# zhuzilin/ring-flash-attention

Measured on AMD Instinct MI355X. Metric: iters/sec fwd+bwd zigzag_ring, seq=8192*ws, h=32, d=128 bf16, higher is better.
Workload: dtype bf16; 1 GPU; zigzag_ring_flash_attn_kvpacked_func fwd+bwd, per-rank q=(1,8192,32,128) kv=(1,8192,2,8,128) bf16 causal, total seq 8192; kv_heads=8, world_size=1, forward_only=False

## Files before the change

ring-flash-attention_amd/csrc/rfa_bwd.hip:

```cpp
#include <type_traits>

#include "rfa_common.hpp"
#include "rfa_kernels.hpp"

#ifndef RFA_DQ_AHEAD1
#define RFA_DQ_AHEAD1 3
#endif
#ifndef RFA_KV_AHEAD
#define RFA_KV_AHEAD 3
#endif
#ifndef RFA_KV_WIDE_UNROLL
#define RFA_KV_WIDE_UNROLL 1
#endif
#ifndef RFA_KV_AHEAD2
#define RFA_KV_AHEAD2 2
#endif
#ifndef RFA_KV_X_LOAD
#define RFA_KV_X_LOAD 1
#endif
#ifndef RFA_KV_X_LDS
#define RFA_KV_X_LDS 1
#endif
#ifndef RFA_KV_X_VALU
#define RFA_KV_X_VALU 1
#endif
#ifndef RFA_KV_X_SYNC
#define RFA_KV_X_SYNC 1
#endif
#ifndef RFA_KV_PRIO
#define RFA_KV_PRIO 0
#endif
#ifndef RFA_SPILL_AUX
#define RFA_SPILL_AUX 2
#endif
#ifndef RFA_KV_PIN
#define RFA_KV_PIN 1
#endif

namespace rfa {

constexpr int kDqWaves = 8;
constexpr int kDqThreads = kDqWaves * 64;
constexpr int kDqRows = kDqWaves * 32;
constexpr int kDqKV = 64;
template <int kD> constexpr int dq_smem() { return 4 * kDqKV * HeadGeo<kD>::kRowBytes; }

template <typename T, int kD, bool kFullD, bool kWin, bool kDrop = false>
__global__ __launch_bounds__(kDqThreads, 2) void dq_kernel(const BwdParams p) {
  extern __shared__ __attribute__((aligned(16))) char smem_raw[];
  lds_t* smem = (lds_t*)smem_raw;
  typedef HeadGeo<kD> Geo;
  constexpr int kRowBytes = Geo::kRowBytes;
  constexpr int kNK = Geo::kKSteps, kNB = Geo::kDBlocks;
  constexpr int kDqTileBytes = kDqKV * kRowBytes;
  constexpr int kShare = kDqTileBytes / 1024 / kDqWaves;
  constexpr int kChunks = Geo::kLay / 8;
  constexpr int kRowsPerPass = kDqThreads / kChunks;

  const int tid = threadIdx.x;
  const int lane = tid & 63;
  const int wave = __builtin_amdgcn_readfirstlane(tid >> 6);
  const int g = lane >> 5;
  const int l31 = lane & 31;

  int idx = blockIdx.x;
  const int G = p.H / p.Hk;
// ... 387 lines not shown
    const int kr = krow < lk ? krow : lk - 1;
    const T* kp = kbase + (int64_t)kr * p.k_st.row;
#pragma unroll
    for (int kk = 0; kk < kNK; ++kk) {
      const int chunk = 2 * kk + g;
      kwr[kk] = (kFullD || chunk * 8 < p.D) ? *(const vec8<T>*)(kp + chunk * 8) : zero8<T>();
    }
  }

  vec8<T> qreg[kPasses], doreg[kPasses];
  float statreg = 0.f;
  const float stat_scale = (tid & kKvQ) ? -1.f : -kLog2e;
#ifndef RFA_KV_DMA
#define RFA_KV_DMA 1
#endif
  constexpr bool kDma = kFullD && RFA_KV_DMA;
  int voff_q[kPasses], voff_do[kPasses];
#pragma unroll
  for (int i = 0; i < kPasses; ++i) {
    int row = sr + kRowsPerPass * i, chunk = sc;
    if (kDma) dma_lane_src<kD>(wave + kKvWaves * i, lane, row, chunk);
    voff_q[i] = (row * (int)p.q_st.row + chunk * 8) * 2;
    voff_do[i] = (row * (int)p.dout_st.row + chunk * 8) * 2;
  }
  int dma_stage = 0;
  int ld_g = 0, ld_j = jtop > 0 ? jtop : 0;
  int ld_c = 0;
  const int64_t q_tile_e = (int64_t)kKvQ * p.q_st.row, do_tile_e = (int64_t)kKvQ * p.dout_st.row;
  const float* st_base0 = wave ? dltbase0 : lsebase0;
  const int64_t st_head_e = wave ? p.delta_head : p.lse_head;
  const T* ld_q = qbase0 + ld_j * q_tile_e;
  const T* ld_do = dobase0 + ld_j * do_tile_e;
  const float* ld_st = st_base0 + ld_j * kKvQ;
  auto load_tile = [&]() {
    const int j = RFA_KV_X_LOAD == 2 ? 0 : ld_j;
    const T* qtile = RFA_KV_X_LOAD == 2 ? qbase0 : ld_q;
    const T* dotile = RFA_KV_X_LOAD == 2 ? dobase0 : ld_do;
    const float* sttile = ld_st;
    if (++ld_g >= G) {
      ld_g = 0;
      if (kBal) {
        ++ld_c;
        ld_j = ld_c == w_n1 ? w_j2 : (ld_c < w_n1 ? ld_j - 1 : ld_j + 1);
      } else {
        ld_j -= nsplit;
      }
      ld_q = qbase0 + ld_j * q_tile_e;
      ld_do = dobase0 + ld_j * do_tile_e;
      ld_st = st_base0 + ld_j * kKvQ;
    } else {
      ld_q += p.q_st.head;
      ld_do += p.dout_st.head;
      ld_st += st_head_e;
    }
    int rows = lq - j * kKvQ;
    rows = rows < kKvQ ? rows : kKvQ;
    const int nq = rows > 0 ? ((rows - 1) * (int)p.q_st.row + p.D) * 2 : 0;
    const int ndo = rows > 0 ? ((rows - 1) * (int)p.dout_st.row + p.D) * 2 : 0;
    const buf_rsrc_t rq = make_rsrc(qtile, nq);
    const buf_rsrc_t rdo = make_rsrc(dotile, ndo);
    const dma_rsrc_t dq_ = make_dma_rsrc(qtile, nq);
    const dma_rsrc_t ddo = make_dma_rsrc(dotile, ndo);
#pragma unroll
    for (int i = 0; i < kPasses; ++i) {
      if (kDma) {
        const int dst = lds_addr(smem) + dma_stage + (wave + kKvWaves * i) * 1024;
        dma_load128(dq_, dst, voff_q[i]);
        if (RFA_KV_X_LOAD != 3) dma_load128(ddo, dst + kOffDo, voff_do[i]);
      } else {
        qreg[i] = buffer_load128<T>(rq, voff_q[i]);
        doreg[i] = buffer_load128<T>(rdo, voff_do[i]);
        if (!sd_ok) {
          qreg[i] = zero8<T>();
          doreg[i] = zero8<T>();
        }
      }
    }
    if (wave < 2) {
      const dma_rsrc_t rs = make_dma_rsrc(sttile, rows > 0 ? rows * 4 : 0);
      statreg = buffer_load32_async(rs, lane * 4);
    }
    dma_stage ^= kKvTileBytes;
  };
  int wq = lds_addr(smem) + tile_off_d<kD>(sr, sc);
  int ws = lds_addr(smem) + kOffStat + tid * 4;
  auto write_tile = [&]() {
    if (!kDma) {
#pragma unroll
      for (int i = 0; i < kPasses; ++i) {
        lds_write128<T>(lds_ptr(wq) + i * kRowsPerPass * kRowBytes, qreg[i]);
        lds_write128<T>(lds_ptr(wq) + i * kRowsPerPass * kRowBytes + kOffDo, doreg[i]);
      }
    }
    if (tid < 2 * kKvQ) *(__attribute__((address_space(3))) float*)lds_ptr(ws) = statreg * stat_scale;
  };

  int aq = lds_addr(smem) + tile_off_d<kD>(l31, g) + par * 32 * kRowBytes;
  const int av = lds_addr(smem) + tile_off_d<kD>(l31, g) + kOffV + kbw * 32 * kRowBytes;
  int tq[kTK][2];
#pragma unroll
  for (int kv = 0; kv < kTK; ++kv)
#pragma unroll
    for (int hh = 0; hh < 2; ++hh) {
      tq[kv][hh] = lds_addr(smem) + par * 32 * kRowBytes + tr_off_d<kD>(lane, 0, 16 * kv + 8 * hh + 4 * g);
      pin_vgpr(tq[kv][hh]);
    }
  int mask_g4 = 4 * g, mask_kg = krow - 4 * g;
  pin_vgpr(mask_g4); pin_vgpr(mask_kg);
  int sa = lds_addr(smem) + kOffStat + (32 * par + 4 * g) * 4;
  int avp = av;
  pin_vgpr(aq); pin_vgpr(avp); pin_vgpr(sa); pin_vgpr(wq); pin_vgpr(ws);

  const int ds_lane = 16 * (16 * (l31 >> 2) + 4 * g + (l31 & 3));
  const int ds_nkb = ds_blocks(p.Sk, p.k_half);
  const int64_t ds_head_bytes = p.ds_head_blocks * kDsBlockBytes;
  const char* ds_b = kSpill ? (const char*)p.ds + ds_base_blocks(p, b) * kDsBlockBytes + (int64_t)h0 * ds_head_bytes : nullptr;
  const int64_t ds_g0 = (qs.row0 >> 5) + b;
  const int ds_kb = __builtin_amdgcn_readfirstlane(kblk * (kKeys / 32) + kbw);

  const uint32_t drop_j = kDrop ? p.k_pos0 + (uint32_t)(p.cu_k ? ks.row0 : 0) + (uint32_t)krow : 0u;
  const uint32_t drop_i0 = kDrop ? p.q_pos0 + (uint32_t)(p.cu_q ? qs.row0 : 0) : 0u;
  const float c = p.scale * kLog2e;
  f32x16 dk[kNB], dv[kNB];
#pragma unroll
  for (int i = 0; i < kNB; ++i)
#pragma unroll
    for (int r = 0; r < 16; ++r) { dk[i][r] = 0.f; dv[i][r] = 0.f; }

  load_tile();
  wait_all_vmem();
  load_landed(statreg);
  write_tile();
  wq ^= kKvTileBytes;
  ws ^= kKvStatBytes;
  __syncthreads();

#if RFA_KV_PRIO == 1
  if (par == 0) __builtin_amdgcn_s_setprio(2);
#elif RFA_KV_PRIO == 2
  if (wave >= kKvWaves / 2) __builtin_amdgcn_s_setprio(1);
#endif
  const int ntile = ntile_q * G;
  int j = jtop, cg = 0, jc = 0;
  int ds_roff0 = kSpill ? (int)ds_rowpart(p, 2 * j, ds_g0, ds_nkb) : 0;
  int ds_rlen0 = kSpill ? ds_rowlen(p, 2 * j, ds_nkb) : 0;
  const char* ds_hp = ds_b;
  for (int f = 0; f < ntile; ++f) {
    if (RFA_KV_X_LOAD && f + 1 < ntile) load_tile();
    int nact = 0;
    bool active = false;
#if RFA_KV_WIDE_UNROLL
#pragma unroll
#else
#pragma unroll 1
#endif
    for (int t0 = 0; t0 < (kWide ? 2 : 1); ++t0) {
    const int t = kWide ? t0 : par;
    constexpr bool kImm = kWide && RFA_KV_WIDE_UNROLL;
    const int toff = kImm ? t0 * 32 * kRowBytes : 0, soff_t = kImm ? t0 * 32 * 4 : 0;
    const int qs0 = j * kKvQ + 32 * t;
    active = (kw0 < lk) && (qs0 < lq) && !(hi && qs0 + 31 + off + wr < kw0) &&
             !(lo && qs0 + off - wl > kw0 + 31);
    if (active) {
      ++nact;
      f32x16 s, dp;
      if (RFA_KV_PRIO == 3 || RFA_KV_PRIO == 5) __builtin_amdgcn_s_setprio(1);
#pragma unroll
      for (int jj = 0; jj < 4; ++jj) {
        const f32x4 nd = *(__attribute__((address_space(3))) f32x4*)(lds_ptr(sa) + (kKvQ + 8 * jj) * 4 + soff_t);
#pragma unroll
        for (int e = 0; e < 4; ++e) { dp[4 * jj + e] = nd[e]; s[4 * jj + e] = 0.f; }
      }
      {
        constexpr int kAhead = RFA_KV_AHEAD;
        constexpr int kN = 2 * kNK;
        vec8<T> a[kN], w[kNK];
        auto fa = [&](int i) {
          if (!RFA_KV_X_LDS || (RFA_KV_X_LDS == 2 && t0 == 1)) return kwr[i % kNK];
          return lds_read128<T>(lds_ptr(aq ^ ((i % kNK) << 5)) + (i < kNK ? kOffDo : 0) + toff);
        };
        auto fw = [&](int i) {
          if (!RFA_KV_X_LDS || (RFA_KV_X_LDS == 2 && t0 == 1)) return kwr[i];
          return lds_read128<T>(lds_ptr(avp ^ (i << 5)));
        };
#pragma unroll
        for (int i = 0; i < kAhead; ++i) { a[i] = fa(i); w[i] = fw(i); }
#pragma unroll
        for (int i = 0; i < kN; ++i) {
          if (i + kAhead < kN) a[i + kAhead] = fa(i + kAhead);
          if (i + kAhead < kNK) w[i + kAhead] = fw(i + kAhead);
          if (i < kNK) dp = mfma(a[i], w[i], dp);
          else s = mfma(a[i], kwr[i - kNK], s);
// ... 6 lines not shown
          __builtin_amdgcn_sched_group_barrier(0x100, 2, 0);
        }
#pragma unroll
        for (int i = 0; i < kNK; ++i) {
          __builtin_amdgcn_sched_group_barrier(0x008, 1, 0);
          __builtin_amdgcn_sched_group_barrier(0x100, 1, 0);
        }
        __builtin_amdgcn_sched_group_barrier(0x008, kAhead, 0);
#endif
      }
      if (RFA_KV_PRIO == 3 || RFA_KV_PRIO == 5) __builtin_amdgcn_s_setprio(0);
      f32x4 l2v[4];
#pragma unroll
      for (int jj = 0; jj < 4; ++jj) l2v[jj] = *(__attribute__((address_space(3))) f32x4*)(lds_ptr(sa) + 8 * jj * 4 + soff_t);
      const bool need_mask = (qs0 + 32 > lq) || (hi && qs0 + off + wr < kw0 + 31) ||
                             (lo && qs0 + 31 + off - wl > kw0);
#pragma unroll
      for (int jj = 0; jj < 4; ++jj)
#pragma unroll
        for (int e = 0; e < 4; ++e)
          if (RFA_KV_X_VALU) s[4 * jj + e] = fast_exp2(__builtin_fmaf(s[4 * jj + e], c, l2v[jj][e]));
      if (RFA_KV_X_VALU && need_mask) {
#pragma unroll
        for (int r = 0; r < 16; ++r) {
          const int sq = qs0 + crow(r, 0);
          const bool ok = (mask_g4 < lq - sq) & (!hi | (mask_kg <= sq + off + wr)) & (!lo | (mask_kg >= sq + off - wl));
          s[r] = ok ? s[r] : 0.f;
        }
      }
      if (kDrop) {
        const uint32_t hkey = drop_head_key(p.drop_seed, p.cu_q ? 0u : (uint32_t)b, p.head0 + (uint32_t)(h0 + cg));
#pragma unroll
        for (int jj = 0; jj < 4; ++jj) {
          const f32x4 nd = *(__attribute__((address_space(3))) f32x4*)(lds_ptr(sa) + (kKvQ + 8 * jj) * 4);
#pragma unroll
          for (int e = 0; e < 4; ++e) {
            const int r = 4 * jj + e;
            const uint32_t w = drop_word(hkey, drop_i0 + (uint32_t)(qs0 + crow(r, g)), drop_j >> 2);
            const bool keep = drop_keep(w, (int)(drop_j & 3u), p.drop_keep);
            const float dpd = keep ? (dp[r] - nd[e]) * p.drop_scale + nd[e] : nd[e];
            dp[r] = dpd * s[r];
            s[r] = keep ? s[r] * p.drop_scale : 0.f;
          }
        }
      } else {
#pragma unroll
      for (int jj = 0; jj < 4; ++jj)
#pragma unroll
        for (int e = 0; e < 4; ++e)
          if (RFA_KV_X_VALU) dp[4 * jj + e] *= s[4 * jj + e];
      }
      {
        const vec8<T> pb0 = pack8<T>(s, 0), pb1 = pack8<T>(s, 8);
        const vec8<T> ds0 = pack8<T>(dp, 0), ds1 = pack8<T>(dp, 8);
#ifndef RFA_SPILL_PROBE
#define RFA_SPILL_PROBE 0
#endif
        auto spill = [&]() {
          if (!kSpill || RFA_SPILL_PROBE == 1) return;
          unsigned boff = (unsigned)(ds_roff0 + (t ? ds_rlen0 : 0) + ds_kb) * (unsigned)kDsBlockBytes;
          if (RFA_SPILL_PROBE == 4) boff = (unsigned)(blockIdx.x * 8 + wave) * (unsigned)kDsBlockBytes;
          const buf_rsrc_t rb = make_rsrc(RFA_SPILL_PROBE == 4 ? (const char*)p.ds : ds_hp, -1);
          __builtin_amdgcn_raw_buffer_store_b128(__builtin_bit_cast(u32x4, ds0), rb, ds_lane, (int)boff, RFA_SPILL_AUX);
          if (RFA_SPILL_PROBE != 3)
            __builtin_amdgcn_raw_buffer_store_b128(__builtin_bit_cast(u32x4, ds1), rb, ds_lane + 128, (int)boff, RFA_SPILL_AUX);
        };
        if (RFA_SPILL_PROBE != 2) spill();
// ... 21 lines not shown
          else dk[dblk] = mfma(a[i], ks2 ? ds1 : ds0, dk[dblk]);
        }
#if RFA_KV_PIN
        __builtin_amdgcn_sched_group_barrier(0x100, 2 * kAhead, 1);
#pragma unroll
        for (int i = 0; i < kN2 - kAhead; ++i) {
          __builtin_amdgcn_sched_group_barrier(0x008, 1, 1);
          __builtin_amdgcn_sched_group_barrier(0x100, 2, 1);
        }
        __builtin_amdgcn_sched_group_barrier(0x008, kAhead, 1);
#endif
        if (RFA_KV_PRIO == 4 || RFA_KV_PRIO == 5) __builtin_amdgcn_s_setprio(0);
        if (RFA_SPILL_PROBE == 2) spill();
      }
    }
    if (kWide && !kImm) {
      aq ^= 32 * kRowBytes;
#pragma unroll
      for (int kv = 0; kv < kTK; ++kv) {
        tq[kv][0] ^= 32 * kRowBytes;
        tq[kv][1] ^= 32 * kRowBytes;
      }
      sa ^= 32 * 4;
    }
    }
    if (!RFA_KV_X_SYNC) {
    } else if (kWide && kSpill && nact == 2) wait_vmem<4>();
    else if (kWide && kSpill && nact == 1) wait_vmem<2>();
    else if (kWide) wait_all_vmem();
    else if (kSpill && active && RFA_SPILL_PROBE != 1 && RFA_SPILL_PROBE != 3) wait_vmem<2>();
    else if (kSpill && active && RFA_SPILL_PROBE == 3) wait_vmem<1>();
    else wait_all_vmem();
    load_landed(statreg);
    if (f + 1 < ntile) write_tile();
    if (++cg >= G) {
      cg = 0;
      if (kBal) {
        ++jc;
        j = jc == w_n1 ? w_j2 : (jc < w_n1 ? j - 1 : j + 1);
      } else {
        j -= nsplit;
      }
      if (kSpill) {
        ds_roff0 = (int)ds_rowpart(p, 2 * j, ds_g0, ds_nkb);
        ds_rlen0 = ds_rowlen(p, 2 * j, ds_nkb);
        ds_hp = ds_b;
      }
    } else if (kSpill) {
      ds_hp += ds_head_bytes;
    }
    aq ^= kKvTileBytes;
#pragma unroll
    for (int kv = 0; kv < kTK; ++kv) {
      tq[kv][0] ^= kKvTileBytes;
      tq[kv][1] ^= kKvTileBytes;
    }
    sa ^= kKvStatBytes;
    wq ^= kKvTileBytes;
    ws ^= kKvStatBytes;
    if (RFA_KV_X_SYNC) __syncthreads();
  }

  if (!kWide) {
    float* xbuf = (float*)smem_raw;
    constexpr int kXW = kNB * 1024;
    const int slot = (par == 1 ? 0 : 4 * kXW) + kbw * kXW;
    const f32x16(&mine)[kNB] = (par == 1) ? dk : dv;
#pragma unroll
    for (int dblk = 0; dblk < kNB; ++dblk)
#pragma unroll
      for (int r = 0; r < 16; ++r) xbuf[slot + (dblk * 16 + r) * 64 + lane] = mine[dblk][r];
    __syncthreads();
    const int rslot = (par == 0 ? 0 : 4 * kXW) + kbw * kXW;
    f32x16(&fin)[kNB] = (par == 0) ? dk : dv;
#pragma unroll
    for (int dblk = 0; dblk < kNB; ++dblk)
#pragma unroll
      for (int r = 0; r < 16; ++r) fin[dblk][r] += xbuf[rslot + (dblk * 16 + r) * 64 + lane];
  }

  bool do_final = true, add_partner = false;
  const __attribute__((address_space(1))) char* pair_src = nullptr;
  if (kBal && !(bal_b && seg == 0)) {
    typedef __attribute__((address_space(1))) unsigned gu32;
    const int64_t pid = ((int64_t)b * p.Hk + hk) * bal_half + bal_j;
    gu32* flag = (gu32*)(p.pair_flags + pid);
    __attribute__((address_space(3))) unsigned* role_w = (__attribute__((address_space(3))) unsigned*)(smem + kOffStat);
    if (tid == 0) {
      unsigned seen = 0u;
      __hip_atomic_compare_exchange_strong(flag, &seen, 1u, __ATOMIC_RELAXED, __ATOMIC_RELAXED, __HIP_MEMORY_SCOPE_AGENT);
      *role_w = seen;
    }
    __syncthreads();
// ... 204 lines not shown
```

ring-flash-attention_amd/csrc/rfa_common.hpp:

```cpp
#pragma once
#include <hip/hip_runtime.h>
#include <stdint.h>

namespace rfa {

typedef __bf16 bf16_t;
typedef _Float16 f16_t;

template <typename T> using vec8 = T __attribute__((ext_vector_type(8)));
template <typename T> using vec4 = T __attribute__((ext_vector_type(4)));
template <typename T> using vec2 = T __attribute__((ext_vector_type(2)));
typedef float f32x16 __attribute__((ext_vector_type(16)));
typedef float f32x4 __attribute__((ext_vector_type(4)));
typedef float f32x2 __attribute__((ext_vector_type(2)));
typedef short s16x4 __attribute__((ext_vector_type(4)));
typedef int i32x4 __attribute__((ext_vector_type(4)));
typedef unsigned int u32x4 __attribute__((ext_vector_type(4)));
typedef int i32x2 __attribute__((ext_vector_type(2)));

typedef __attribute__((address_space(3))) char lds_t;

constexpr int kHeadDim = 128;
constexpr int kRowBytes = kHeadDim * 2;
constexpr float kLog2e = 1.4426950408889634f;
// ... 202 lines not shown
}
__device__ __forceinline__ float buffer_load32_async(dma_rsrc_t r, int voffset) {
  float v;
  asm volatile("s_nop 4\n\tbuffer_load_dword %0, %1, %2, 0 offen" : "=v"(v) : "v"(voffset), "s"(r.w));
  return v;
}
__device__ __forceinline__ void load_landed(float& v) { asm volatile("" : "+v"(v)); }
__device__ __forceinline__ float buffer_load32(buf_rsrc_t r, int voffset) {
  return __builtin_bit_cast(float, __builtin_amdgcn_raw_buffer_load_b32(r, voffset, 0, 0));
}

__host__ __device__ __forceinline__ uint32_t fmix32(uint32_t x) {
  x ^= x >> 16; x *= 0x85EBCA6Bu; x ^= x >> 13; x *= 0xC2B2AE35u; x ^= x >> 16;
  return x;
}
__host__ __device__ __forceinline__ uint32_t drop_head_key(uint64_t seed, uint32_t batch, uint32_t head) {
  return fmix32((uint32_t)seed ^ fmix32((uint32_t)(seed >> 32) ^ fmix32(head * 0x27D4EB2Fu ^ fmix32(batch + 0x165667B1u))));
}
__device__ __forceinline__ uint32_t drop_word(uint32_t head_key, uint32_t i, uint32_t jq) {
  return fmix32((i * 0x9E3779B1u) ^ (jq * 0x85EBCA77u) ^ head_key);
}
__device__ __forceinline__ bool drop_keep(uint32_t word, int byte, uint32_t keep) {
  return ((word >> (8 * byte)) & 0xffu) < keep;
}

__device__ __forceinline__ float shfl_xor32(float v) { return __shfl_xor(v, 32, 64); }
__device__ __forceinline__ float max_xor32(float v) {
  const unsigned u = __builtin_bit_cast(unsigned, v);
  auto r = __builtin_amdgcn_permlane32_swap(u, u, false, false);
  float d;
  asm("v_max_f32 %0, %1, %2" : "=v"(d) : "v"((unsigned)r[0]), "v"((unsigned)r[1]));
  return d;
}
__device__ __forceinline__ float sum_xor32(float v) {
  const unsigned u = __builtin_bit_cast(unsigned, v);
  auto r = __builtin_amdgcn_permlane32_swap(u, u, false, false);
  return __builtin_bit_cast(float, (unsigned)r[0]) + __builtin_bit_cast(float, (unsigned)r[1]);
}

__device__ __forceinline__ float fast_exp2(float x) { return __builtin_amdgcn_exp2f(x); }

}
```

ring-flash-attention_amd/csrc/rfa_fwd.hip:

```cpp
#include <type_traits>

#include "rfa_common.hpp"
#include "rfa_kernels.hpp"

#ifndef RFA_FWD_DEFER
#define RFA_FWD_DEFER 8
#endif
#ifndef RFA_FWD_AHEAD
#define RFA_FWD_AHEAD 6
#endif
#ifndef RFA_FWD_AHEAD_V
#define RFA_FWD_AHEAD_V 3
#endif
#ifndef RFA_FWD_LEAN
#define RFA_FWD_LEAN 1
#endif
#ifndef RFA_FWD_MAXFORM
#define RFA_FWD_MAXFORM 1
#endif
#ifndef RFA_FWD_PACKED_VALU
#define RFA_FWD_PACKED_VALU 0
#endif

namespace rfa {

#ifndef RFA_FWD_X_LOAD
#define RFA_FWD_X_LOAD 1
#endif
constexpr int kFwdWavesMax = 8;
#ifndef RFA_FWD_KV
#define RFA_FWD_KV 64
#endif
#ifndef RFA_FWD_YOUNG_PRIO
#define RFA_FWD_YOUNG_PRIO 0
#endif
constexpr int kFwdKV = RFA_FWD_KV;
constexpr int kFwdSub = kFwdKV / 32;
#ifndef RFA_FWD_STAGES
#define RFA_FWD_STAGES 2
#endif
constexpr int kFwdStages = RFA_FWD_STAGES;
template <int kD> constexpr int fwd_smem() { return 2 * kFwdStages * kFwdKV * HeadGeo<kD>::kRowBytes; }

template <typename T, int kD, bool kFullD, bool kWin, bool kDrop = false, int kW = kFwdWavesMax>
__global__ __launch_bounds__(kW * 64, 2) void fwd_kernel(const FwdParams p) {
  constexpr int kFwdWaves = kW, kFwdThreads = kW * 64, kFwdQRows = kW * 32;
  extern __shared__ __attribute__((aligned(16))) char smem_raw[];
  lds_t* smem = (lds_t*)smem_raw;
  typedef HeadGeo<kD> Geo;
  constexpr int kRowBytes = Geo::kRowBytes;
  constexpr int kNK = Geo::kKSteps, kNB = Geo::kDBlocks;
// ... 149 lines not shown
  const uint32_t drop_j0 = kDrop ? p.k_pos0 + (uint32_t)(p.cu_k ? ks.row0 : 0) : 0u;
  const float c = p.scale * kLog2e;
  float m = -INFINITY;
  float mthr = -INFINITY, mc_run = 0.f;
  float lsum = 0.f;
  f32x16 o[kNB];
#pragma unroll
  for (int i = 0; i < kNB; ++i)
#pragma unroll
    for (int r = 0; r < 16; ++r) o[i][r] = 0.f;

  constexpr int kDist = kDma ? kFwdStages - 1 : 1;
  load_tile(jt0, std::integral_constant<int, 0>{});
  write_tile(std::integral_constant<int, 0>{});
  wait_all_vmem();
  __syncthreads();
  if (kDist == 2) load_tile(jt0 + 1, std::integral_constant<int, 1>{});
#if RFA_FWD_YOUNG_PRIO
  if (wave >= kFwdWaves / 2) __builtin_amdgcn_s_setprio(1);
#endif

  auto tile_step = [&](int j, auto stage) {
    constexpr int kStage = decltype(stage)::value;
    constexpr int kbo = kStage * kFwdTileBytes;
    constexpr int vbo = kStage * kFwdTileBytes;
    typedef std::integral_constant<int, (kStage + kDist) % kFwdStages> fill_t;
    typedef std::integral_constant<int, (kStage + 1) % kFwdStages> next_t;
    const bool more = j + kDist < ntiles;
    if (more) load_tile(j + kDist, fill_t{});

    const int kt0 = j * kFwdKV;
    const bool active = (qw0 < lq) && !(hi && kt0 > qw0 + 31 + off + wr) &&
                        !(lo && kt0 + kFwdKV - 1 < qw0 + off - wl);
    if (active) {
      f32x16 s[kFwdSub];
#pragma unroll
      for (int t = 0; t < kFwdSub; ++t)
#pragma unroll
        for (int r = 0; r < 16; ++r) s[t][r] = 0.f;
      {
        constexpr int kAhead = RFA_FWD_AHEAD;
        constexpr int kN = kFwdSub * kNK;
        vec8<T> a[kN];
        auto fa = [&](int i) { return lds_read128<T>(lds_ptr(koff[i % kNK]) + kbo + (i / kNK) * 32 * kRowBytes); };
#pragma unroll
        for (int i = 0; i < kAhead; ++i) a[i] = fa(i);
#pragma unroll
        for (int i = 0; i < kN; ++i) {
          if (i + kAhead < kN) a[i + kAhead] = fa(i + kAhead);
          s[i / kNK] = mfma(a[i], qf[i % kNK], s[i / kNK]);
        }
        __builtin_amdgcn_sched_group_barrier(0x100, kAhead, 0);
#pragma unroll
        for (int i = 0; i < kN - kAhead; ++i) {
          __builtin_amdgcn_sched_group_barrier(0x008, 1, 0);
          __builtin_amdgcn_sched_group_barrier(0x100, 1, 0);
        }
        __builtin_amdgcn_sched_group_barrier(0x008, kAhead, 0);
      }
      const bool need_mask = (kt0 + kFwdKV > lk) || (hi && kt0 + kFwdKV - 1 > qw0 + off + wr) ||
                             (lo && kt0 < qw0 + 31 + off - wl);
      if (need_mask) {
        const int lim = hi ? ((qrow + off + wr < lk - 1) ? qrow + off + wr : lk - 1) : lk - 1;
        const int lim_lo = lo ? qrow + off - wl : -0x40000000;
#pragma unroll
        for (int t = 0; t < kFwdSub; ++t)
#pragma unroll
          for (int r = 0; r < 16; ++r) {
            const int key = kt0 + 32 * t + crow(r, g);
            if (key > lim || (kWin && key < lim_lo)) s[t][r] = -INFINITY;
          }
      }
      float mloc = s[0][0];
#pragma unroll
      for (int r = 1; r < 16; ++r) mloc = fmaxf(mloc, s[0][r]);
#pragma unroll
      for (int t = 1; t < kFwdSub; ++t)
#pragma unroll
        for (int r = 0; r < 16; ++r) mloc = fmaxf(mloc, s[t][r]);
      mloc = RFA_FWD_MAXFORM ? max_xor32(mloc) : fmaxf(mloc, shfl_xor32(mloc));
      bool rescale = true;
      if (RFA_FWD_LEAN) {
        rescale = !__all(mloc <= mthr);
      } else {
        const float mnew0 = fmaxf(m, mloc);
        if (RFA_FWD_DEFER > 0) rescale = !__all((mnew0 - m) * c <= (float)RFA_FWD_DEFER);
      }
      if (rescale) {
        const float mnew = fmaxf(m, mloc);
        const float msafe = (mnew == -INFINITY) ? 0.f : mnew;
        const float alpha = fast_exp2(m * c - msafe * c);
        m = mnew;
        mc_run = msafe * c;
        mthr = mnew + (RFA_FWD_DEFER > 0 ? (float)RFA_FWD_DEFER / c : 0.f);
        lsum *= alpha;
#pragma unroll
        for (int i = 0; i < kNB; ++i)
#pragma unroll
          for (int r = 0; r < 16; ++r) o[i][r] *= alpha;
      }
      const float mc = RFA_FWD_LEAN ? mc_run : ((m == -INFINITY) ? 0.f : m) * c;
#if RFA_FWD_PACKED_VALU
      f32x16 psum16;
#pragma unroll
      for (int t = 0; t < kFwdSub; ++t) {
        s[t] = s[t] * c - mc;
#pragma unroll
        for (int r = 0; r < 16; ++r) s[t][r] = fast_exp2(s[t][r]);
        psum16 = t ? psum16 + s[t] : s[t];
      }
      f32x4 ps4;
#pragma unroll
      for (int e = 0; e < 4; ++e) ps4[e] = (psum16[e] + psum16[4 + e]) + (psum16[8 + e] + psum16[12 + e]);
      lsum += (ps4[0] + ps4[1]) + (ps4[2] + ps4[3]);
#else
      float psum = 0.f;
#pragma unroll
      for (int t = 0; t < kFwdSub; ++t)
#pragma unroll
        for (int r = 0; r < 16; ++r) {
          const float pv = fast_exp2(__builtin_fmaf(s[t][r], c, -mc));
          s[t][r] = pv;
          psum += pv;
        }
      lsum += psum;
#endif
      if (kDrop) {
        const int mis = __builtin_amdgcn_readfirstlane((int)(drop_j0 & 3u));
#pragma unroll
        for (int t = 0; t < kFwdSub; ++t)
#pragma unroll
          for (int mm = 0; mm < 4; ++mm) {
            const uint32_t jg = drop_j0 + (uint32_t)(kt0 + 32 * t + 8 * mm + 4 * g);
            uint32_t w = drop_word(drop_key, drop_i, jg >> 2);
            if (mis) w = __builtin_amdgcn_alignbyte(drop_word(drop_key, drop_i, (jg >> 2) + 1), w, (uint32_t)mis);
#pragma unroll
            for (int e = 0; e < 4; ++e)
              if (!drop_keep(w, e, p.drop_keep)) s[t][4 * mm + e] = 0.f;
          }
      }

#pragma unroll
      for (int t = 0; t < kFwdSub; ++t)
#pragma unroll
        for (int ks2 = 0; ks2 < 2; ++ks2) {
          const vec8<T> pb = pack8<T>(s[t], 8 * ks2);
          constexpr int kPer = Geo::kSwzRows;
          const int rows = 32 * t + 16 * ks2;
          const int imm = vbo + (rows / kPer) * kPer * kRowBytes;
          const int kv = (rows % kPer) / 16;
#pragma unroll
          for (int dblk = 0; dblk < kNB; ++dblk) {
            vec4<T> lo = lds_read_tr<T>(lds_ptr(voff[dblk][kv][0]) + imm);
            vec4<T> hi = lds_read_tr<T>(lds_ptr(voff[dblk][kv][1]) + imm);
            o[dblk] = mfma(concat<T>(lo, hi), pb, o[dblk]);
          }
        }
    }
    if (!kDma && more) write_tile(next_t{});
    if (kDma) {
      if (kDist == 2 && more) wait_vmem<2 * kFwdShare>();
      else wait_all_vmem();
    }
    __syncthreads();
  };
  if (kFwdStages == 3) {
    for (int j = jt0; j < ntiles; j += 3) {
      tile_step(j, std::integral_constant<int, 0>{});
      if (j + 1 < ntiles) tile_step(j + 1, std::integral_constant<int, 1>{});
      if (j + 2 < ntiles) tile_step(j + 2, std::integral_constant<int, 2 % kFwdStages>{});
    }
  } else {
    for (int j = jt0; j < ntiles; j += 2) {
      tile_step(j, std::integral_constant<int, 0>{});
      if (j + 1 < ntiles) tile_step(j + 1, std::integral_constant<int, 1>{});
    }
  }

  if (qrow >= lq) return;
  const float l = RFA_FWD_MAXFORM ? sum_xor32(lsum) : lsum + shfl_xor32(lsum);
  const bool has = l > 0.f;
  const float inv = has ? (kDrop ? p.drop_scale : 1.f) / l : 0.f;
  const float blse = has ? m * p.scale + __logf(l) : INFINITY;
  const int64_t orow = qs.row0 + qrow;

  if (p.out_acc == nullptr && nsplit == 1) {
    T* ob = (T*)p.out + qbatch * p.out_st.batch + orow * p.out_st.row + (int64_t)h * p.out_st.head;
    store_rows16<T, kFullD, kNB>(ob, o, inv, g, p.D, true);
    if (g == 0) p.lse[qbatch * p.lse_batch + (int64_t)h * p.lse_head + orow] = blse;
  } else {
// ... 158 lines not shown
  int s0 = 0;

  for (int pass = 0;; ++pass) {
    Item nxt;
    const bool has_next = item_at(pass + 1, nxt);
    const T *nkb = kb, *nvb = vb;
    if (has_next) kv_base(nxt, nkb, nvb);
    const int ntiles = cur.ntiles;
    const T *run_k = kb + k_tile_e, *run_v = vb + v_tile_e;
    const int qw0 = cur.qwg0 + wave * 32;
    const int qrow = qw0 + l31;

    float m = -INFINITY, mthr = -INFINITY, mc_run = 0.f, lsum = 0.f;
    f32x16 o[kNB];
#pragma unroll
    for (int i = 0; i < kNB; ++i)
#pragma unroll
      for (int r = 0; r < 16; ++r) o[i][r] = 0.f;

    auto tile_step = [&](int j, auto stage) {
      constexpr int kStage = decltype(stage)::value;
      constexpr int kbo = kStage * kTileBytes, vbo = kStage * kTileBytes;
      const bool last = j + 1 >= ntiles;
      if (!last || has_next) {
        const int jn = last ? 0 : j + 1;
        int rows = lk - jn * kFwdKV;
        rows = rows < kFwdKV ? rows : kFwdKV;
        dma_rows(last ? nkb : run_k, last ? nvb : run_v, rows, kStage ^ 1);
        run_k += k_tile_e;
        run_v += v_tile_e;
      }
      const int kt0 = j * kFwdKV;
      const bool active = (qw0 < lq) && !(hi && kt0 > qw0 + 31 + off);
      if (active) {
        f32x16 s[kFwdSub];
#pragma unroll
        for (int t = 0; t < kFwdSub; ++t)
#pragma unroll
          for (int r = 0; r < 16; ++r) s[t][r] = 0.f;
        {
        constexpr int kAhead = RFA_FWD_AHEAD;
        constexpr int kN = kFwdSub * kNK;
        vec8<T> a[kN];
        auto fa = [&](int i) { return lds_read128<T>(lds_ptr(koff[i % kNK]) + kbo + (i / kNK) * 32 * kRowBytes); };
#pragma unroll
        for (int i = 0; i < kAhead; ++i) a[i] = fa(i);
#pragma unroll
        for (int i = 0; i < kN; ++i) {
          if (i + kAhead < kN) a[i + kAhead] = fa(i + kAhead);
          s[i / kNK] = mfma(a[i], qf[i % kNK], s[i / kNK]);
        }
        __builtin_amdgcn_sched_group_barrier(0x100, kAhead, 0);
#pragma unroll
        for (int i = 0; i < kN - kAhead; ++i) {
          __builtin_amdgcn_sched_group_barrier(0x008, 1, 0);
          __builtin_amdgcn_sched_group_barrier(0x100, 1, 0);
        }
        __builtin_amdgcn_sched_group_barrier(0x008, kAhead, 0);
        }
        const bool need_mask = (kt0 + kFwdKV > lk) || (hi && kt0 + kFwdKV - 1 > qw0 + off);
        if (need_mask) {
          const int lim = hi ? ((qrow + off < lk - 1) ? qrow + off : lk - 1) : lk - 1;
#pragma unroll
          for (int t = 0; t < kFwdSub; ++t)
#pragma unroll
            for (int r = 0; r < 16; ++r) {
              const int key = kt0 + 32 * t + crow(r, g);
              if (key > lim) s[t][r] = -INFINITY;
            }
        }
        float mloc = s[0][0];
#pragma unroll
        for (int r = 1; r < 16; ++r) mloc = fmaxf(mloc, s[0][r]);
#pragma unroll
        for (int t = 1; t < kFwdSub; ++t)
#pragma unroll
          for (int r = 0; r < 16; ++r) mloc = fmaxf(mloc, s[t][r]);
        mloc = max_xor32(mloc);
        if (!__all(mloc <= mthr)) {
          const float mnew = fmaxf(m, mloc);
          const float msafe = (mnew == -INFINITY) ? 0.f : mnew;
          const float alpha = fast_exp2(m * c - msafe * c);
          m = mnew;
          mc_run = msafe * c;
          mthr = mnew + (RFA_FWD_DEFER > 0 ? (float)RFA_FWD_DEFER / c : 0.f);
          lsum *= alpha;
#pragma unroll
          for (int i = 0; i < kNB; ++i)
#pragma unroll
            for (int r = 0; r < 16; ++r) o[i][r] *= alpha;
        }
        const float mc = mc_run;
        float psum = 0.f;
#pragma unroll
        for (int t = 0; t < kFwdSub; ++t)
#pragma unroll
          for (int r = 0; r < 16; ++r) {
            const float pv = fast_exp2(__builtin_fmaf(s[t][r], c, -mc));
            s[t][r] = pv;
            psum += pv;
          }
        lsum += psum;
        {
          vec8<T> pb[2 * kFwdSub];
#pragma unroll
          for (int x = 0; x < 2 * kFwdSub; ++x) pb[x] = pack8<T>(s[x >> 1], 8 * (x & 1));
          constexpr int kNV = 2 * kFwdSub * kNB;
          constexpr int kAheadV = RFA_FWD_AHEAD_V;
          vec8<T> va[kNV];
          auto fv = [&](int i) {
            const int dblk = i % kNB, x = i / kNB;
            const int imm = vbo + 16 * x * kRowBytes;
            return concat<T>(lds_read_tr<T>(lds_ptr(voff[dblk][0]) + imm), lds_read_tr<T>(lds_ptr(voff[dblk][1]) + imm));
          };
#pragma unroll
          for (int i = 0; i < kAheadV; ++i) va[i] = fv(i);
#pragma unroll
          for (int i = 0; i < kNV; ++i) {
            if (i + kAheadV < kNV) va[i + kAheadV] = fv(i + kAheadV);
            o[i % kNB] = mfma(va[i], pb[i / kNB], o[i % kNB]);
          }
          __builtin_amdgcn_sched_group_barrier(0x100, 2 * kAheadV, 1);
#pragma unroll
          for (int i = 0; i < kNV - kAheadV; ++i) {
            __builtin_amdgcn_sched_group_barrier(0x008, 1, 1);
            __builtin_amdgcn_sched_group_barrier(0x100, 2, 1);
          }
          __builtin_amdgcn_sched_group_barrier(0x008, kAheadV, 1);
        }
      }
      if (!last) {
        wait_all_vmem();
        __syncthreads();
      }
    };
    int j = 0;
    if (s0) {
      tile_step(0, std::integral_constant<int, 1>{});
      j = 1;
    }
    for (; j < ntiles; j += 2) {
      tile_step(j, std::integral_constant<int, 0>{});
      if (j + 1 < ntiles) tile_step(j + 1, std::integral_constant<int, 1>{});
    }

    if (has_next) load_q(nxt);
    {
      const float l = sum_xor32(lsum);
      const bool has = l > 0.f;
      const float inv = has ? 1.f / l : 0.f;
      const float blse = has ? m * p.scale + __logf(l) : INFINITY;
      int rows = lq - qw0;
      rows = rows < 32 ? (rows > 0 ? rows : 0) : 32;
      T* ob = (T*)p.out + (int64_t)cur.b * p.out_st.batch + (qs.row0 + qw0) * p.out_st.row + (int64_t)cur.h * p.out_st.head;
      const buf_rsrc_t ro = make_rsrc(rows > 0 ? ob : (T*)p.out, rows > 0 ? ((rows - 1) * (int)p.out_st.row + kD) * 2 : 0);
      const int ll = opaque_lane();
      const int vo = ((ll & 31) * (int)p.out_st.row + 8 * (ll >> 5)) * 2;
#pragma unroll
      for (int dblk = 0; dblk < kNB; ++dblk)
#pragma unroll
        for (int mm = 0; mm < 2; ++mm) {
// ... 89 lines not shown
```

Baseline: 508.4 iters/sec.

## Skip dead causal sub-tiles in fwd, unroll bwd KV stages, add max3 option

The forward kernels now check whether the second 32-key sub-block of a KV tile is entirely masked, either by the causal diagonal or by running past the key length. When it is, they run a specialised one-sub-block body, so the QK MFMAs, exp and PV MFMAs for that half are skipped. The backward dK/dV kernel unrolls its double-buffered tile loop by two so the LDS stage offsets become compile-time immediates instead of per-iteration pointer XORs, which adds code size and register pressure. A v_max3-based row-max path is also added but is off by default.

Result: slower. 495.8 iters/sec (-2.5%).

```diff
diff --git a/ring-flash-attention_amd/csrc/rfa_bwd.hip b/ring-flash-attention_amd/csrc/rfa_bwd.hip
--- a/ring-flash-attention_amd/csrc/rfa_bwd.hip
+++ b/ring-flash-attention_amd/csrc/rfa_bwd.hip
@@ -32,6 +32,9 @@
 #endif
 #ifndef RFA_SPILL_AUX
 #define RFA_SPILL_AUX 2
+#endif
+#ifndef RFA_KV_STAGE_UNROLL
+#define RFA_KV_STAGE_UNROLL 1
 #endif
 #ifndef RFA_KV_PIN
 #define RFA_KV_PIN 1
@@ -485,7 +488,8 @@
   const T* ld_q = qbase0 + ld_j * q_tile_e;
   const T* ld_do = dobase0 + ld_j * do_tile_e;
   const float* ld_st = st_base0 + ld_j * kKvQ;
-  auto load_tile = [&]() {
+  auto load_tile = [&](auto stage) {
+    constexpr int kFill = decltype(stage)::value;
     const int j = RFA_KV_X_LOAD == 2 ? 0 : ld_j;
     const T* qtile = RFA_KV_X_LOAD == 2 ? qbase0 : ld_q;
     const T* dotile = RFA_KV_X_LOAD == 2 ? dobase0 : ld_do;
@@ -517,7 +521,7 @@
 #pragma unroll
     for (int i = 0; i < kPasses; ++i) {
       if (kDma) {
-        const int dst = lds_addr(smem) + dma_stage + (wave + kKvWaves * i) * 1024;
+        const int dst = lds_addr(smem) + (kFill < 0 ? dma_stage : kFill * kKvTileBytes) + (wave + kKvWaves * i) * 1024;
         dma_load128(dq_, dst, voff_q[i]);
         if (RFA_KV_X_LOAD != 3) dma_load128(ddo, dst + kOffDo, voff_do[i]);
       } else {
@@ -533,19 +537,21 @@
       const dma_rsrc_t rs = make_dma_rsrc(sttile, rows > 0 ? rows * 4 : 0);
       statreg = buffer_load32_async(rs, lane * 4);
     }
-    dma_stage ^= kKvTileBytes;
+    if (kFill < 0) dma_stage ^= kKvTileBytes;
   };
   int wq = lds_addr(smem) + tile_off_d<kD>(sr, sc);
   int ws = lds_addr(smem) + kOffStat + tid * 4;
-  auto write_tile = [&]() {
+  auto write_tile = [&](auto stage) {
+    constexpr int kTo = decltype(stage)::value;
+    constexpr int qo = kTo > 0 ? kTo * kKvTileBytes : 0, so = kTo > 0 ? kTo * kKvStatBytes : 0;
     if (!kDma) {
 #pragma unroll
       for (int i = 0; i < kPasses; ++i) {
-        lds_write128<T>(lds_ptr(wq) + i * kRowsPerPass * kRowBytes, qreg[i]);
-        lds_write128<T>(lds_ptr(wq) + i * kRowsPerPass * kRowBytes + kOffDo, doreg[i]);
-      }
-    }
-    if (tid < 2 * kKvQ) *(__attribute__((address_space(3))) float*)lds_ptr(ws) = statreg * stat_scale;
+        lds_write128<T>(lds_ptr(wq) + i * kRowsPerPass * kRowBytes + qo, qreg[i]);
+        lds_write128<T>(lds_ptr(wq) + i * kRowsPerPass * kRowBytes + kOffDo + qo, doreg[i]);
+      }
+    }
+    if (tid < 2 * kKvQ) *(__attribute__((address_space(3))) float*)(lds_ptr(ws) + so) = statreg * stat_scale;
   };
 
   int aq = lds_addr(smem) + tile_off_d<kD>(l31, g) + par * 32 * kRowBytes;
@@ -580,12 +586,16 @@
 #pragma unroll
     for (int r = 0; r < 16; ++r) { dk[i][r] = 0.f; dv[i][r] = 0.f; }
 
-  load_tile();
+  constexpr bool kStageImm = RFA_KV_STAGE_UNROLL != 0;
+  typedef std::integral_constant<int, kStageImm ? 0 : -1> stage0_t;
+  load_tile(stage0_t{});
   wait_all_vmem();
   load_landed(statreg);
-  write_tile();
-  wq ^= kKvTileBytes;
-  ws ^= kKvStatBytes;
+  write_tile(stage0_t{});
+  if (!kStageImm) {
+    wq ^= kKvTileBytes;
+    ws ^= kKvStatBytes;
+  }
   __syncthreads();
 
 #if RFA_KV_PRIO == 1
@@ -598,8 +608,16 @@
   int ds_roff0 = kSpill ? (int)ds_rowpart(p, 2 * j, ds_g0, ds_nkb) : 0;
   int ds_rlen0 = kSpill ? ds_rowlen(p, 2 * j, ds_nkb) : 0;
   const char* ds_hp = ds_b;
-  for (int f = 0; f < ntile; ++f) {
-    if (RFA_KV_X_LOAD && f + 1 < ntile) load_tile();
+  auto tile_step = [&](int f, auto stage) {
+    constexpr int kStage = decltype(stage)::value;
+    constexpr int st_q = kStage > 0 ? kStage * kKvTileBytes : 0, st_s = kStage > 0 ? kStage * kKvStatBytes : 0;
+    typedef std::integral_constant<int, kStage < 0 ? -1 : (kStage ^ 1)> fill_t;
+    if (RFA_KV_X_LOAD && f + 1 < ntile) load_tile(fill_t{});
+    if (kStage >= 0) {
+      pin_vgpr(aq);
+#pragma unroll
+      for (int kv = 0; kv < kTK; ++kv) { pin_vgpr(tq[kv][0]); pin_vgpr(tq[kv][1]); }
+    }
     int nact = 0;
     bool active = false;
 #if RFA_KV_WIDE_UNROLL
@@ -610,7 +628,7 @@
     for (int t0 = 0; t0 < (kWide ? 2 : 1); ++t0) {
     const int t = kWide ? t0 : par;
     constexpr bool kImm = kWide && RFA_KV_WIDE_UNROLL;
-    const int toff = kImm ? t0 * 32 * kRowBytes : 0, soff_t = kImm ? t0 * 32 * 4 : 0;
+    const int toff = (kImm ? t0 * 32 * kRowBytes : 0) + st_q, soff_t = (kImm ? t0 * 32 * 4 : 0) + st_s;
     const int qs0 = j * kKvQ + 32 * t;
     active = (kw0 < lk) && (qs0 < lq) && !(hi && qs0 + 31 + off + wr < kw0) &&
              !(lo && qs0 + off - wl > kw0 + 31);
@@ -683,7 +701,7 @@
         const uint32_t hkey = drop_head_key(p.drop_seed, p.cu_q ? 0u : (uint32_t)b, p.head0 + (uint32_t)(h0 + cg));
 #pragma unroll
         for (int jj = 0; jj < 4; ++jj) {
-          const f32x4 nd = *(__attribute__((address_space(3))) f32x4*)(lds_ptr(sa) + (kKvQ + 8 * jj) * 4);
+          const f32x4 nd = *(__attribute__((address_space(3))) f32x4*)(lds_ptr(sa) + (kKvQ + 8 * jj) * 4 + st_s);
 #pragma unroll
           for (int e = 0; e < 4; ++e) {
             const int r = 4 * jj + e;
@@ -771,7 +789,7 @@
     else if (kSpill && active && RFA_SPILL_PROBE == 3) wait_vmem<1>();
     else wait_all_vmem();
     load_landed(statreg);
-    if (f + 1 < ntile) write_tile();
+    if (f + 1 < ntile) write_tile(fill_t{});
     if (++cg >= G) {
       cg = 0;
       if (kBal) {
@@ -788,16 +806,26 @@
     } else if (kSpill) {
       ds_hp += ds_head_bytes;
     }
-    aq ^= kKvTileBytes;
-#pragma unroll
-    for (int kv = 0; kv < kTK; ++kv) {
-      tq[kv][0] ^= kKvTileBytes;
-      tq[kv][1] ^= kKvTileBytes;
-    }
-    sa ^= kKvStatBytes;
-    wq ^= kKvTileBytes;
-    ws ^= kKvStatBytes;
+    if (kStage < 0) {
+      aq ^= kKvTileBytes;
+#pragma unroll
+      for (int kv = 0; kv < kTK; ++kv) {
+        tq[kv][0] ^= kKvTileBytes;
+        tq[kv][1] ^= kKvTileBytes;
+      }
+      sa ^= kKvStatBytes;
+      wq ^= kKvTileBytes;
+      ws ^= kKvStatBytes;
+    }
     if (RFA_KV_X_SYNC) __syncthreads();
+  };
+  if (kStageImm) {
+    for (int f = 0; f < ntile; f += 2) {
+      tile_step(f, std::integral_constant<int, 0>{});
+      if (f + 1 < ntile) tile_step(f + 1, std::integral_constant<int, 1>{});
+    }
+  } else {
+    for (int f = 0; f < ntile; ++f) tile_step(f, std::integral_constant<int, -1>{});
   }
 
   if (!kWide) {
diff --git a/ring-flash-attention_amd/csrc/rfa_common.hpp b/ring-flash-attention_amd/csrc/rfa_common.hpp
--- a/ring-flash-attention_amd/csrc/rfa_common.hpp
+++ b/ring-flash-attention_amd/csrc/rfa_common.hpp
@@ -258,6 +258,18 @@
   asm("v_max_f32 %0, %1, %2" : "=v"(d) : "v"((unsigned)r[0]), "v"((unsigned)r[1]));
   return d;
 }
+__device__ __forceinline__ float max3_asm(float a, float b, float c) {
+  float d;
+  asm("v_max3_f32 %0, %1, %2, %3" : "=v"(d) : "v"(a), "v"(b), "v"(c));
+  return d;
+}
+template <int kN>
+__device__ __forceinline__ float row_max3(const f32x16 (&s)[kN]) {
+  float m = __builtin_amdgcn_fmed3f(s[kN - 1][14], s[kN - 1][15], INFINITY);
+#pragma unroll
+  for (int i = 0; i < 16 * kN - 2; i += 2) m = max3_asm(m, s[i / 16][i % 16], s[i / 16][i % 16 + 1]);
+  return m;
+}
 __device__ __forceinline__ float sum_xor32(float v) {
   const unsigned u = __builtin_bit_cast(unsigned, v);
   auto r = __builtin_amdgcn_permlane32_swap(u, u, false, false);
diff --git a/ring-flash-attention_amd/csrc/rfa_fwd.hip b/ring-flash-attention_amd/csrc/rfa_fwd.hip
--- a/ring-flash-attention_amd/csrc/rfa_fwd.hip
+++ b/ring-flash-attention_amd/csrc/rfa_fwd.hip
@@ -17,6 +17,12 @@
 #endif
 #ifndef RFA_FWD_MAXFORM
 #define RFA_FWD_MAXFORM 1
+#endif
+#ifndef RFA_FWD_MAX3
+#define RFA_FWD_MAX3 0
+#endif
+#ifndef RFA_FWD_SUBSKIP
+#define RFA_FWD_SUBSKIP 1
 #endif
 #ifndef RFA_FWD_PACKED_VALU
 #define RFA_FWD_PACKED_VALU 0
@@ -232,15 +238,16 @@
     const int kt0 = j * kFwdKV;
     const bool active = (qw0 < lq) && !(hi && kt0 > qw0 + 31 + off + wr) &&
                         !(lo && kt0 + kFwdKV - 1 < qw0 + off - wl);
-    if (active) {
-      f32x16 s[kFwdSub];
-#pragma unroll
-      for (int t = 0; t < kFwdSub; ++t)
+    auto body = [&](auto nsub) {
+      constexpr int kSub = decltype(nsub)::value;
+      f32x16 s[kSub];
+#pragma unroll
+      for (int t = 0; t < kSub; ++t)
 #pragma unroll
         for (int r = 0; r < 16; ++r) s[t][r] = 0.f;
       {
         constexpr int kAhead = RFA_FWD_AHEAD;
-        constexpr int kN = kFwdSub * kNK;
+        constexpr int kN = kSub * kNK;
         vec8<T> a[kN];
         auto fa = [&](int i) { return lds_read128<T>(lds_ptr(koff[i % kNK]) + kbo + (i / kNK) * 32 * kRowBytes); };
 #pragma unroll
@@ -264,20 +271,25 @@
         const int lim = hi ? ((qrow + off + wr < lk - 1) ? qrow + off + wr : lk - 1) : lk - 1;
         const int lim_lo = lo ? qrow + off - wl : -0x40000000;
 #pragma unroll
-        for (int t = 0; t < kFwdSub; ++t)
+        for (int t = 0; t < kSub; ++t)
 #pragma unroll
           for (int r = 0; r < 16; ++r) {
             const int key = kt0 + 32 * t + crow(r, g);
             if (key > lim || (kWin && key < lim_lo)) s[t][r] = -INFINITY;
           }
       }
-      float mloc = s[0][0];
-#pragma unroll
-      for (int r = 1; r < 16; ++r) mloc = fmaxf(mloc, s[0][r]);
-#pragma unroll
-      for (int t = 1; t < kFwdSub; ++t)
-#pragma unroll
-        for (int r = 0; r < 16; ++r) mloc = fmaxf(mloc, s[t][r]);
+      float mloc;
+      if (RFA_FWD_MAX3) {
+        mloc = row_max3(s);
+      } else {
+        mloc = s[0][0];
+#pragma unroll
+        for (int r = 1; r < 16; ++r) mloc = fmaxf(mloc, s[0][r]);
+#pragma unroll
+        for (int t = 1; t < kSub; ++t)
+#pragma unroll
+          for (int r = 0; r < 16; ++r) mloc = fmaxf(mloc, s[t][r]);
+      }
       mloc = RFA_FWD_MAXFORM ? max_xor32(mloc) : fmaxf(mloc, shfl_xor32(mloc));
       bool rescale = true;
       if (RFA_FWD_LEAN) {
@@ -303,7 +315,7 @@
 #if RFA_FWD_PACKED_VALU
       f32x16 psum16;
 #pragma unroll
-      for (int t = 0; t < kFwdSub; ++t) {
+      for (int t = 0; t < kSub; ++t) {
         s[t] = s[t] * c - mc;
 #pragma unroll
         for (int r = 0; r < 16; ++r) s[t][r] = fast_exp2(s[t][r]);
@@ -316,7 +328,7 @@
 #else
       float psum = 0.f;
 #pragma unroll
-      for (int t = 0; t < kFwdSub; ++t)
+      for (int t = 0; t < kSub; ++t)
 #pragma unroll
         for (int r = 0; r < 16; ++r) {
           const float pv = fast_exp2(__builtin_fmaf(s[t][r], c, -mc));
@@ -328,7 +340,7 @@
       if (kDrop) {
         const int mis = __builtin_amdgcn_readfirstlane((int)(drop_j0 & 3u));
 #pragma unroll
-        for (int t = 0; t < kFwdSub; ++t)
+        for (int t = 0; t < kSub; ++t)
 #pragma unroll
           for (int mm = 0; mm < 4; ++mm) {
             const uint32_t jg = drop_j0 + (uint32_t)(kt0 + 32 * t + 8 * mm + 4 * g);
@@ -341,7 +353,7 @@
       }
 
 #pragma unroll
-      for (int t = 0; t < kFwdSub; ++t)
+      for (int t = 0; t < kSub; ++t)
 #pragma unroll
         for (int ks2 = 0; ks2 < 2; ++ks2) {
           const vec8<T> pb = pack8<T>(s[t], 8 * ks2);
@@ -356,6 +368,16 @@
             o[dblk] = mfma(concat<T>(lo, hi), pb, o[dblk]);
           }
         }
+    };
+    const bool tail_dead = RFA_FWD_SUBSKIP && kFullD && !kDrop && kFwdSub == 2 && ((hi && kt0 + 32 > qw0 + 31 + off + wr) || kt0 + 32 >= lk);
+    if (active) {
+      if (tail_dead) {
+        asm volatile("" ::: "memory");
+        body(std::integral_constant<int, 1>{});
+        asm volatile("" ::: "memory");
+      } else {
+        body(std::integral_constant<int, kFwdSub>{});
+      }
     }
     if (!kDma && more) write_tile(next_t{});
     if (kDma) {
@@ -580,15 +602,16 @@
       }
       const int kt0 = j * kFwdKV;
       const bool active = (qw0 < lq) && !(hi && kt0 > qw0 + 31 + off);
-      if (active) {
-        f32x16 s[kFwdSub];
-#pragma unroll
-        for (int t = 0; t < kFwdSub; ++t)
+      auto body = [&](auto nsub) {
+        constexpr int kSub = decltype(nsub)::value;
+        f32x16 s[kSub];
+#pragma unroll
+        for (int t = 0; t < kSub; ++t)
 #pragma unroll
           for (int r = 0; r < 16; ++r) s[t][r] = 0.f;
         {
         constexpr int kAhead = RFA_FWD_AHEAD;
-        constexpr int kN = kFwdSub * kNK;
+        constexpr int kN = kSub * kNK;
         vec8<T> a[kN];
         auto fa = [&](int i) { return lds_read128<T>(lds_ptr(koff[i % kNK]) + kbo + (i / kNK) * 32 * kRowBytes); };
 #pragma unroll
@@ -610,20 +633,25 @@
         if (need_mask) {
           const int lim = hi ? ((qrow + off < lk - 1) ? qrow + off : lk - 1) : lk - 1;
 #pragma unroll
-          for (int t = 0; t < kFwdSub; ++t)
+          for (int t = 0; t < kSub; ++t)
 #pragma unroll
             for (int r = 0; r < 16; ++r) {
               const int key = kt0 + 32 * t + crow(r, g);
               if (key > lim) s[t][r] = -INFINITY;
             }
         }
-        float mloc = s[0][0];
-#pragma unroll
-        for (int r = 1; r < 16; ++r) mloc = fmaxf(mloc, s[0][r]);
-#pragma unroll
-        for (int t = 1; t < kFwdSub; ++t)
-#pragma unroll
-          for (int r = 0; r < 16; ++r) mloc = fmaxf(mloc, s[t][r]);
+        float mloc;
+        if (RFA_FWD_MAX3) {
+          mloc = row_max3(s);
+        } else {
+          mloc = s[0][0];
+#pragma unroll
+          for (int r = 1; r < 16; ++r) mloc = fmaxf(mloc, s[0][r]);
+#pragma unroll
+          for (int t = 1; t < kSub; ++t)
+#pragma unroll
+            for (int r = 0; r < 16; ++r) mloc = fmaxf(mloc, s[t][r]);
+        }
         mloc = max_xor32(mloc);
         if (!__all(mloc <= mthr)) {
           const float mnew = fmaxf(m, mloc);
@@ -641,7 +669,7 @@
         const float mc = mc_run;
         float psum = 0.f;
 #pragma unroll
-        for (int t = 0; t < kFwdSub; ++t)
+        for (int t = 0; t < kSub; ++t)
 #pragma unroll
           for (int r = 0; r < 16; ++r) {
             const float pv = fast_exp2(__builtin_fmaf(s[t][r], c, -mc));
@@ -650,10 +678,10 @@
           }
         lsum += psum;
         {
-          vec8<T> pb[2 * kFwdSub];
-#pragma unroll
-          for (int x = 0; x < 2 * kFwdSub; ++x) pb[x] = pack8<T>(s[x >> 1], 8 * (x & 1));
-          constexpr int kNV = 2 * kFwdSub * kNB;
+          vec8<T> pb[2 * kSub];
+#pragma unroll
+          for (int x = 0; x < 2 * kSub; ++x) pb[x] = pack8<T>(s[x >> 1], 8 * (x & 1));
+          constexpr int kNV = 2 * kSub * kNB;
           constexpr int kAheadV = RFA_FWD_AHEAD_V;
           vec8<T> va[kNV];
           auto fv = [&](int i) {
@@ -675,6 +703,16 @@
             __builtin_amdgcn_sched_group_barrier(0x100, 2, 1);
           }
           __builtin_amdgcn_sched_group_barrier(0x008, kAheadV, 1);
+        }
+      };
+      const bool tail_dead = RFA_FWD_SUBSKIP && ((hi && kt0 + 32 > qw0 + 31 + off) || kt0 + 32 >= lk);
+      if (active) {
+        if (tail_dead) {
+          asm volatile("" ::: "memory");
+          body(std::integral_constant<int, 1>{});
+          asm volatile("" ::: "memory");
+        } else {
+          body(std::integral_constant<int, kFwdSub>{});
         }
       }
       if (!last) {
```
